# DanielPS555/Radix-sort-Merge-Sort-CUDA---Lab-y-practicos-GPGPU-2023

Hardware: AMD Instinct MI355X
Metric: Mkeys/s sorting uint32, n=2^28, 1 GPU (+ merge-sort at 2/4/8) (higher is better)
Workload: dtype u32; 1 GPU; LSD radix sort (8-bit digits, onesweep), n=2^28 uint32 u32, device-resident (BASELINE config 3); n_per_gpu=268435456, algo=radix, key=u32, dist=u32, parallelism=single GPU

## Files before the change

### radix-sort-merge-sort-cuda---lab-y-practicos-gpgpu-2023_amd/csrc/api.hip

```cpp
#include <hip/hip_runtime.h>

#include <algorithm>
#include <cstdio>
#include <cstdlib>
#include <cstring>
#include <mutex>
#include <vector>

#include "host.h"
#include "segsort.h"

using namespace labsort;

namespace {

thread_local int g_last_hip = 0;

struct TimedLaunch {
    int cls;
    hipEvent_t a, b;
};
std::mutex g_timing_mu;
bool g_timing_on = false;
std::vector<TimedLaunch> g_pending;
// ... 100 lines not shown

bool use_gather(size_t n) {
    const char *e = std::getenv("LABSORT_RADIX_IMPL");
    if (e && !std::strcmp(e, "gather")) return true;
    if (n < GS_MIN_N || n >= GS_MAX_N) return false;
    return !(e && !std::strcmp(e, "onesweep"));
}

uint32_t hybrid_gate(size_t n) {
    const char *e = std::getenv("LABSORT_RADIX_HYBRID");
    if (e && !std::strcmp(e, "0")) return 0u;
    if (e && !std::strcmp(e, "2")) return HY_MAX_BUCKET;
    return n >= HY_MIN_N && n <= HY_MAX_N ? HY_FAST_GROUP : 0u;
}

uint32_t hy_count_mode() {
    const char *e = std::getenv("LABSORT_HY_COUNT");
    if (e && !std::strcmp(e, "lean")) return HY_COUNT_LEAN;
    if (e && !std::strcmp(e, "full")) return HY_COUNT_FULL;
    return HY_COUNT_AUTO;
}

bool small_path(size_t n, int algo) { return algo != LABSORT_ALGO_RADIX1 && n <= (size_t)TS_TILE; }

int sort_radix8(const uint32_t *ki, const uint32_t *vi, uint32_t *ko, uint32_t *vo, size_t n, uint32_t flip, char *ws,
                hipStream_t s) {
    const RadixLayout L = radix_layout(n, 8, OSP_TILE);
    Bufs b, vb;
    b.p[SEL_IN] = const_cast<uint32_t *>(ki);
    b.p[SEL_OUT] = ko;
    b.p[SEL_TMP] = reinterpret_cast<uint32_t *>(ws + L.off_tmp);
    vb.p[SEL_IN] = const_cast<uint32_t *>(vi);
    vb.p[SEL_OUT] = vo;
    vb.p[SEL_TMP] = vi ? reinterpret_cast<uint32_t *>(ws + align_up(L.total, 256)) : nullptr;
    uint32_t *hist = reinterpret_cast<uint32_t *>(ws + L.off_hist);
    uint32_t *counters = reinterpret_cast<uint32_t *>(ws + L.off_counter);
    uint32_t *err = reinterpret_cast<uint32_t *>(ws + L.off_err);
    uint32_t *lookback = reinterpret_cast<uint32_t *>(ws + L.off_lookback);
    Plan *plan = reinterpret_cast<Plan *>(ws + L.off_plan);
    HIP_TRY(launch_zero(ws, L.off_lookback, s));
    uint32_t *hps = reinterpret_cast<uint32_t *>(ws + L.off_hps);
    uint32_t *joint = reinterpret_cast<uint32_t *>(ws + L.off_joint);
    SegPlan *sps = reinterpret_cast<SegPlan *>(ws + L.off_segplan);
    const uint32_t hy_limit = vi ? 0u : hybrid_gate(n);
    const bool hyb = hy_limit != 0u;
    const HyCounts hc{reinterpret_cast<uint32_t *>(ws + L.off_hps2), reinterpret_cast<uint32_t *>(ws + L.off_top14), hy_limit,
                      err, hy_count_mode()};
    {
        TimingScope ts(LABSORT_K_HISTOGRAM, s);
        if (hyb) HIP_TRY(launch_hist_lean(ki, n, flip, joint, s, hc));
        HIP_TRY(launch_hist_seg(ki, n, flip, hps, joint, s, hyb ? &hc : nullptr));
    }
    HIP_TRY(launch_plan8(hps, joint, n, ki == ko ? 1 : 0, plan, sps, hist, ws + L.off_lookback,
                         L.zero_bytes - L.off_lookback, s, hyb ? &hc : nullptr));
    for (int p = 0; p < L.P; ++p) {
        TimingScope ts(hyb && p < 2 ? LABSORT_K_UNTIMED : LABSORT_K_ONESWEEP, s);
        HIP_TRY(launch_onesweep_p(b, plan, p, n, flip, sps + p, lookback + (size_t)p * L.ntiles * L.R,
                                  counters + (size_t)p * OSP_NCTR, err, s, vi ? &vb : nullptr));
    }
    if (hyb) {
        TimingScope ts(LABSORT_K_SEGSORT, s);
        HIP_TRY(launch_hybrid_finish(plan, b, n, flip, hist, sps + 3, lookback + (size_t)3 * L.ntiles * L.R, L.ntiles, err,
                                     reinterpret_cast<uint32_t *>(ws + L.off_fin_hdr),
                                     reinterpret_cast<uint32_t *>(ws + L.off_fin_off),
                                     reinterpret_cast<uint32_t *>(ws + L.off_fin_lists), s));
    }
    if (ki == ko) {
        HIP_TRY(launch_final_copy(b, plan, n, s));
        if (vi) HIP_TRY(launch_final_copy(vb, plan, n, s));
    }
    return LABSORT_OK;
}

int sort_radix1(const uint32_t *in, uint32_t *out, size_t n, uint32_t flip, char *ws, hipStream_t s) {
    const RadixLayout L = radix_layout(n, 1, OS_TILE);
    Bufs b;
    b.p[SEL_IN] = const_cast<uint32_t *>(in);
    b.p[SEL_OUT] = out;
    b.p[SEL_TMP] = reinterpret_cast<uint32_t *>(ws + L.off_tmp);
    uint32_t *hist = reinterpret_cast<uint32_t *>(ws + L.off_hist);
    uint32_t *counters = reinterpret_cast<uint32_t *>(ws + L.off_counter);
    uint32_t *err = reinterpret_cast<uint32_t *>(ws + L.off_err);
    uint32_t *lookback = reinterpret_cast<uint32_t *>(ws + L.off_lookback);
    Plan *plan = reinterpret_cast<Plan *>(ws + L.off_plan);
    HIP_TRY(launch_zero(ws, L.zero_bytes, s));
    {
        TimingScope ts(LABSORT_K_HISTOGRAM, s);
        HIP_TRY(launch_histogram(in, n, flip, 1, hist, s));
    }
    HIP_TRY(launch_plan(hist, n, 1, in == out ? 1 : 0, plan, s));
    for (int p = 0; p < L.P; ++p) {
        TimingScope ts(LABSORT_K_ONESWEEP, s);
        HIP_TRY(launch_onesweep(b, plan, p, 1, n, flip, hist, lookback + (size_t)p * L.ntiles * L.R,
                                counters + (size_t)p * OSP_NCTR, err, s));
    }
    HIP_TRY(launch_final_copy(b, plan, n, s));
    return LABSORT_OK;
}

int sort_merge(const uint32_t *ki, const uint32_t *vi, uint32_t *ko, uint32_t *vo, size_t n, uint32_t flip, char *ws,
               hipStream_t s) {
    const bool pairs = vi != nullptr;
    const MergeLayout L = merge_layout(n, pairs);
    uint32_t *err = reinterpret_cast<uint32_t *>(ws + L.off_err);
    HIP_TRY(launch_zero(err, 16, s));
    uint32_t *tk = reinterpret_cast<uint32_t *>(ws + L.off_tk);
    uint32_t *tv = pairs ? reinterpret_cast<uint32_t *>(ws + L.off_tv) : nullptr;
// ... 595 lines not shown
```

### radix-sort-merge-sort-cuda---lab-y-practicos-gpgpu-2023_amd/csrc/common.h

```cpp
#pragma once
#include <hip/hip_runtime.h>
#include <stddef.h>
#include <stdint.h>

namespace labsort {

constexpr int WAVE = 64;

__host__ __device__ inline uint32_t f32_ord(uint32_t x) {
    if ((x & 0x7FFFFFFFu) > 0x7F800000u) return 0xFFFFFFFFu;
    return (x & 0x80000000u) ? ~x : x | 0x80000000u;
}
__host__ __device__ inline uint32_t f32_unord(uint32_t o) { return (o & 0x80000000u) ? o & 0x7FFFFFFFu : ~o; }

constexpr uint32_t BF16_NAN_T = 0x7F80u, F16_NAN_T = 0x7C00u;
__host__ __device__ inline uint32_t ord16(uint32_t x, uint32_t nan_t) {
    x &= 0xFFFFu;
    if ((x & 0x7FFFu) > nan_t) return 0xFFFFu;
    return (x & 0x8000u) ? ~x & 0xFFFFu : x | 0x8000u;
}
__host__ __device__ inline uint32_t unord16(uint32_t o) { return (o & 0x8000u) ? o & 0x7FFFu : ~o & 0xFFFFu; }

constexpr int RADIX_BITS = 8;
constexpr int OS_BLOCK = 512;
// ... 81 lines not shown

constexpr int HY_TOP_BITS = 14, HY_TOP = 1 << HY_TOP_BITS;
constexpr uint32_t HY_BUCKETS = 1u << 16;
constexpr uint32_t HY_MAX_BUCKET = 32768;
constexpr size_t HY_MIN_N = ((size_t)1 << 28) - ((size_t)1 << 24);
constexpr size_t HY_MAX_N = ((size_t)1 << 28) + 3 * ((size_t)1 << 24);
constexpr uint32_t HY_FAST_GROUP = 4u * 5120u;
struct HyCounts {
    uint32_t *hps2;
    uint32_t *top14;
    uint32_t limit;
    uint32_t *ctl;
    uint32_t mode;
};
constexpr uint32_t HY_CTL_TICKET = 1;
constexpr uint32_t HY_CTL_NAND = 2;
constexpr uint32_t HY_CTL_OR = 3;
constexpr uint32_t HY_CTL_VERDICT = 4;
constexpr uint32_t HY_CTL_LEAN = 5;
constexpr uint32_t HY_CTL_FULL = 6;
constexpr uint32_t HY_VERDICT_CLASSIC = 1, HY_VERDICT_HYBRID = 2;
constexpr uint32_t HY_COUNT_AUTO = 0, HY_COUNT_LEAN = 1, HY_COUNT_FULL = 2;
#ifndef LABSORT_HY_LEAN_SL
#define LABSORT_HY_LEAN_SL 32
#endif
constexpr int HY_LEAN_SL = LABSORT_HY_LEAN_SL;
inline uint32_t hist_seg_bps(size_t n) {
    const size_t bps = n / ((size_t)NSEG * HS_MIN_KEYS);
    return (uint32_t)(bps < 1 ? 1 : bps > (size_t)HS_BPS ? (size_t)HS_BPS : bps);
}

struct Bufs {
    uint32_t *p[3];
};

constexpr uint32_t LB_AGG = 1u << 30;
constexpr uint32_t LB_INC = 2u << 30;
constexpr uint32_t LB_VAL = (1u << 30) - 1u;
constexpr size_t RADIX_MAX_N = (size_t)LB_VAL;

hipError_t launch_fill(uint32_t *out, size_t n, uint64_t seed, int dist, uint64_t param, uint64_t first,
                       hipStream_t s);
hipError_t launch_histogram(const uint32_t *keys, size_t n, uint32_t flip, int bits, uint32_t *hist,
                            hipStream_t s);
hipError_t launch_plan(const uint32_t *hist, size_t n, int bits, int in_is_out, Plan *plan, hipStream_t s);
hipError_t launch_onesweep(Bufs b, const Plan *plan, int pass, int bits, size_t n, uint32_t flip,
                           const uint32_t *hist, uint32_t *lookback, uint32_t *counter, uint32_t *err,
                           hipStream_t s);
hipError_t launch_hist_seg(const uint32_t *keys, size_t n, uint32_t flip, uint32_t *hps, uint32_t *joint,
                           hipStream_t s, const HyCounts *hy = nullptr);
hipError_t launch_hist_lean(const uint32_t *keys, size_t n, uint32_t flip, uint32_t *joint, hipStream_t s,
                            const HyCounts &hy);
hipError_t launch_plan8(const uint32_t *hps, const uint32_t *joint, size_t n, int in_is_out, Plan *plan,
                        SegPlan *segplans, uint32_t *hist, void *zero_p, size_t zero_bytes, hipStream_t s,
                        const HyCounts *hy = nullptr);
hipError_t launch_onesweep_p(Bufs b, const Plan *plan, int pass, size_t n, uint32_t flip, const SegPlan *sp,
                             uint32_t *lookback, uint32_t *counter, uint32_t *err, hipStream_t s,
                             const Bufs *vb = nullptr);
hipError_t launch_final_copy(Bufs b, const Plan *plan, size_t n, hipStream_t s);
hipError_t launch_tile_sort(const uint32_t *in, uint32_t *out, size_t n, uint32_t flip, hipStream_t s,
                            uint32_t *samp_out = nullptr);
hipError_t launch_wave_tile_sort(uint32_t *keys, size_t n, uint32_t flip, hipStream_t s);
hipError_t launch_merge_pass(const uint32_t *in, uint32_t *out, size_t n, size_t run, uint32_t flip,
                             hipStream_t s, const uint32_t *vin = nullptr, uint32_t *vout = nullptr,
                             const MgPairs *pairs = nullptr, uint32_t *samp_out = nullptr);
hipError_t launch_tile_sort_kv(const uint32_t *in, uint32_t *out, const uint32_t *vin, uint32_t *vout, size_t n,
                               uint32_t flip, hipStream_t s, uint32_t *samp_out = nullptr);
#ifndef LABSORT_M4_S
#define LABSORT_M4_S 128
#endif
constexpr uint32_t M4_S = LABSORT_M4_S;
inline size_t merge4_samp_words(size_t n) { return (n + M4_S - 1) / M4_S + 4; }
size_t merge4_bnd_words(size_t n, size_t r);
hipError_t launch_merge4_pass(const uint32_t *in, uint32_t *out, size_t n, size_t r, uint32_t flip, uint32_t *bnd,
                              const uint32_t *samp_in, uint32_t *samp_out, hipStream_t s, const uint32_t *vin = nullptr,
                              uint32_t *vout = nullptr, uint32_t *err = nullptr);
hipError_t launch_merge_ab(const uint32_t *a, size_t la, const uint32_t *b, size_t lb, uint32_t *out, size_t d0,
                           size_t d1, uint32_t flip, uint32_t *part, hipStream_t s);
hipError_t launch_upper_bound(const uint32_t *keys, size_t n, uint32_t flip, const uint32_t *values, size_t nv,
                              uint32_t *out, hipStream_t s);
struct KeyPrint {
    uint64_t s1, s2, x;
};
bool verify_enabled();
KeyPrint key_print(const int *a, size_t n);
void verify_or_exit(const char *who, const int *a, size_t n, const KeyPrint &before);

hipError_t launch_zero(void *p, size_t bytes, hipStream_t s);
hipError_t launch_stream_copy(const uint32_t *in, uint32_t *out, size_t n, hipStream_t s);
hipError_t launch_f32_map(const uint32_t *in, uint32_t *out, size_t n, bool inverse, hipStream_t s);
hipError_t launch_count_descents(const uint32_t *keys, size_t n, uint32_t flip, uint32_t *count, hipStream_t s);

}
```

### radix-sort-merge-sort-cuda---lab-y-practicos-gpgpu-2023_amd/csrc/fin_block.h

```cpp
#pragma once
#include "segsort.h"

#include "devutil.h"

namespace labsort {

namespace {

#ifndef LABSORT_FIN_PREFETCH
#define LABSORT_FIN_PREFETCH 1
#endif

__device__ __forceinline__ uint32_t wave_incl_scan_dpp(uint32_t x) {
    x += (uint32_t)__builtin_amdgcn_update_dpp(0, (int)x, 0x111, 0xf, 0xf, false);
    x += (uint32_t)__builtin_amdgcn_update_dpp(0, (int)x, 0x112, 0xf, 0xf, false);
    x += (uint32_t)__builtin_amdgcn_update_dpp(0, (int)x, 0x114, 0xf, 0xf, false);
    x += (uint32_t)__builtin_amdgcn_update_dpp(0, (int)x, 0x118, 0xf, 0xf, false);
    x += (uint32_t)__builtin_amdgcn_update_dpp(0, (int)x, 0x142, 0xa, 0xf, false);
    x += (uint32_t)__builtin_amdgcn_update_dpp(0, (int)x, 0x143, 0xc, 0xf, false);
    return x;
}

template <int BLOCK, int KPT>
struct FinSmem {
    static constexpr int R = 256, W = BLOCK / WAVE, TILE = BLOCK * KPT;
    static_assert(TILE <= 65536, "16-bit LDS slots");
    static_assert(W == 4, "the fold holds one counter row per wave in registers");
    uint32_t keys[TILE];
    alignas(16) uint32_t cnt[W * R];
    alignas(16) uint32_t offs[W * R];
    uint32_t probe[WAVE];
    uint32_t ordered;
};

struct FinStripe {
    size_t sb;
    uint32_t ws0;
    uint32_t nf;
    uint32_t ng;
    bool tail_ok;
};
template <int W, int KPT>
__device__ __forceinline__ FinStripe fin_stripe(uint32_t b, uint32_t len, uint32_t lane, uint32_t wid) {
    if (len > (uint32_t)(W * WAVE * KPT)) len = 0u;
    const uint32_t jn = (len + (uint32_t)(W * WAVE) - 1u) / (uint32_t)(W * WAVE);
    const uint32_t ws0 = wid * jn * WAVE;
    const uint32_t rem = ws0 < len ? len - ws0 : 0u;
    const uint32_t nf = min(jn, rem / WAVE);
    const uint32_t tail = nf < jn ? rem - nf * WAVE : 0u;
    return {(size_t)b + ws0, ws0, nf, nf + (tail ? 1u : 0u), lane < tail};
}

template <int KPT>
__device__ __forceinline__ void fin_load(const uint32_t *in, const FinStripe &g, uint32_t lane, uint32_t (&k)[KPT]) {
    const char *pb = reinterpret_cast<const char *>(in + g.sb);
    const uint32_t lb = lane * 4u;
    if (g.nf == (uint32_t)KPT) {
#pragma unroll
        for (int j = 0; j < KPT; ++j) k[j] = ld_stream<NT_TILE>(reinterpret_cast<const uint32_t *>(pb + (lb + (uint32_t)(j * WAVE * 4))));
    } else {
#pragma unroll
        for (int j = 0; j < KPT; ++j) {
            k[j] = 0xFFFFFFFFu;
            if ((uint32_t)j < g.nf || ((uint32_t)j == g.nf && g.tail_ok))
                k[j] = ld_stream<NT_TILE>(reinterpret_cast<const uint32_t *>(pb + (lb + (uint32_t)(j * WAVE * 4))));
        }
    }
}

template <int BLOCK, int KPT>
__device__ __forceinline__ void fin_pass(FinSmem<BLOCK, KPT> &sm, const uint32_t (&k)[KPT], uint32_t shift, uint32_t ng,
                                         bool atomic_rank, uint32_t lane, uint32_t wid) {
    constexpr int W = FinSmem<BLOCK, KPT>::W, R = FinSmem<BLOCK, KPT>::R;
    uint32_t *wh = sm.cnt + wid * R;
    uint32_t *wo = sm.offs + wid * R;
    uint32_t n0 = ng, n1 = ng;
    asm volatile("" : "+s"(n0), "+s"(n1));
    uint32_t z = 0u;
    asm volatile("" : "+v"(z));
    *reinterpret_cast<uint4 *>(wh + 4u * lane) = make_uint4(z, z, z, z);
    uint32_t rank[KPT / 2] = {};
#pragma unroll
    for (int j = 0; j < KPT; ++j) {
        uint32_t r = 0u;
        if ((uint32_t)j < n0) r = rank8(wh, (k[j] >> shift) & 0xFFu, lane, atomic_rank);
        set16(rank, j, r);
    }
    __syncthreads();
    {
        uint4 c[W];
#pragma unroll
        for (int w = 0; w < W; ++w) c[w] = *reinterpret_cast<const uint4 *>(sm.cnt + w * R + 4u * lane);
        uint32_t tot[4] = {0u, 0u, 0u, 0u}, bef[4] = {0u, 0u, 0u, 0u};
#pragma unroll
        for (int w = 0; w < W; ++w) {
            const uint32_t cw[4] = {c[w].x, c[w].y, c[w].z, c[w].w};
            const bool before = (uint32_t)w < wid;
#pragma unroll
            for (int q = 0; q < 4; ++q) {
                tot[q] += cw[q];
                bef[q] += before ? cw[q] : 0u;
            }
        }
        const uint32_t s = tot[0] + tot[1] + tot[2] + tot[3];
        uint32_t run = wave_incl_scan_dpp(s) - s;
        uint4 o4;
        o4.x = run + bef[0];
        run += tot[0];
        o4.y = run + bef[1];
        run += tot[1];
        o4.z = run + bef[2];
        run += tot[2];
        o4.w = run + bef[3];
        *reinterpret_cast<uint4 *>(wo + 4u * lane) = o4;
    }
    __builtin_amdgcn_wave_barrier();
#pragma unroll
    for (int j = 0; j < KPT; ++j)
        if ((uint32_t)j < n1) set16(rank, j, wo[(k[j] >> shift) & 0xFFu] + get16(rank, j));
#pragma unroll
    for (int j = 0; j < KPT; ++j)
        if ((uint32_t)j < n1) sm.keys[get16(rank, j)] = k[j];
    __syncthreads();
}

template <int BLOCK, int KPT, int WPE>
__global__ __launch_bounds__(BLOCK, WPE) void k_fin_block(uint32_t *out, const uint32_t *__restrict__ off,
                                                           const uint32_t *__restrict__ hdr,
                                                           const uint32_t *__restrict__ list, HySel hy) {
    using S = FinSmem<BLOCK, KPT>;
    constexpr int W = S::W;
    constexpr int CLS = 3;
    constexpr bool PREFETCH = LABSORT_FIN_PREFETCH != 0;
    __shared__ S sm;
    if (hy.plan->hybrid == 0u) return;
    const uint32_t *in = hy.buf[hy.plan->fin_src];
    if (ld_agent(hdr) != 0u) return;
    const uint32_t cnt = hdr[SEG_HDR_CNT + CLS];
    const uint32_t tid = threadIdx.x, lane = tid & 63u, wid = __builtin_amdgcn_readfirstlane(tid >> 6);
    if (blockIdx.x >= cnt) return;
    probe_lane_order(sm.probe, &sm.ordered, lane, wid);
    __syncthreads();
    const bool atomic_rank = lane_order_probed(&sm.ordered);
    uint32_t nb, ne;
    {
        const uint32_t seg = __builtin_amdgcn_readfirstlane(list[blockIdx.x]);
        nb = __builtin_amdgcn_readfirstlane(off[seg]);
        ne = __builtin_amdgcn_readfirstlane(off[seg + 1]);
    }
    uint32_t k[KPT];
    FinStripe g = fin_stripe<W, KPT>(nb, ne - nb, lane, wid);
    if constexpr (PREFETCH) fin_load(in, g, lane, k);
    for (uint32_t it = blockIdx.x; it < cnt; it += gridDim.x) {
        if constexpr (!PREFETCH) {
            g = fin_stripe<W, KPT>(nb, ne - nb, lane, wid);
            fin_load(in, g, lane, k);
        }
        const bool more = it + gridDim.x < cnt;
        if (more) {
            const uint32_t seg = __builtin_amdgcn_readfirstlane(list[it + gridDim.x]);
            nb = __builtin_amdgcn_readfirstlane(off[seg]);
            ne = __builtin_amdgcn_readfirstlane(off[seg + 1]);
        }
        fin_pass(sm, k, 0u, g.ng, atomic_rank, lane, wid);
        {
            uint32_t n2 = g.ng;
            asm volatile("" : "+s"(n2));
#pragma unroll
            for (int j = 0; j < KPT; ++j)
                if ((uint32_t)j < n2) k[j] = sm.keys[g.ws0 + (uint32_t)j * WAVE + lane];
        }
        fin_pass(sm, k, 8u, g.ng, atomic_rank, lane, wid);
        FinStripe gn = g;
        uint32_t kn[PREFETCH ? KPT : 1];
        if constexpr (PREFETCH) {
            gn = fin_stripe<W, KPT>(nb, more ? ne - nb : 0u, lane, wid);
            fin_load(in, gn, lane, kn);
        }
        uint32_t nfs = g.nf;
        asm volatile("" : "+s"(nfs));
        const uint32_t *sk = sm.keys + g.ws0 + lane;
        char *ob = reinterpret_cast<char *>(out + g.sb);
        const uint32_t lb = lane * 4u;
        if (nfs == (uint32_t)KPT) {
#pragma unroll
            for (int j = 0; j < KPT; ++j) *reinterpret_cast<uint32_t *>(ob + (lb + (uint32_t)(j * WAVE * 4))) = sk[j * WAVE];
        } else {
#pragma unroll
            for (int j = 0; j < KPT; ++j)
                if ((uint32_t)j < nfs || ((uint32_t)j == nfs && g.tail_ok))
                    *reinterpret_cast<uint32_t *>(ob + (lb + (uint32_t)(j * WAVE * 4))) = sk[j * WAVE];
        }
        if constexpr (PREFETCH) {
            g = gn;
#pragma unroll
            for (int j = 0; j < KPT; ++j) k[j] = kn[j];
        }
    }
}

}

}
```

### radix-sort-merge-sort-cuda---lab-y-practicos-gpgpu-2023_amd/csrc/kernels.hip

```cpp
#include "common.h"
#include "devutil.h"
#include "host.h"
#include "lds_pass.h"

#include <cstdlib>
#include <cstring>
#include <type_traits>

namespace labsort {

__device__ __forceinline__ uint64_t mix64(uint64_t z) {
    z += 0x9E3779B97F4A7C15ull;
    z = (z ^ (z >> 30)) * 0xBF58476D1CE4E5B9ull;
    z = (z ^ (z >> 27)) * 0x94D049BB133111EBull;
    return z ^ (z >> 31);
}

__global__ __launch_bounds__(256) void k_fill(uint32_t *__restrict__ out, size_t n, uint64_t seed, int dist,
                                              uint64_t param, uint64_t first) {
    const size_t stride = (size_t)gridDim.x * blockDim.x;
    for (size_t i = (size_t)blockIdx.x * blockDim.x + threadIdx.x; i < n; i += stride) {
        const uint64_t gi = first + i;
        const uint64_t z = mix64(seed ^ (gi * 0x9E3779B97F4A7C15ull));
        const uint32_t hi = (uint32_t)(z >> 32);
// ... 259 lines not shown
__device__ void build_segplan(SegPlan *__restrict__ sp, const uint32_t *__restrict__ hs, const uint32_t *start,
                              uint32_t mode, uint32_t *sh ) {
    const uint32_t t = threadIdx.x;
    uint32_t tot = 0;
    for (int s = 0; s < NSEG; ++s) {
        const uint32_t v = hs[s * 256 + t];
        sh[s * 256 + t] = v;
        tot += v;
    }
    uint32_t run = block_excl_scan<256, 256>(tot, sh + NSEG * 256);
    for (int s = 0; s < NSEG; ++s) {
        sp->base[s * 256 + t] = run;
        run += sh[s * 256 + t];
    }
    if (t <= (uint32_t)NSEG) sp->start[t] = start[t];
    if (t == 0) {
        uint32_t tp = 0, mx = 0;
        for (int s = 0; s <= NSEG; ++s) {
            sp->tpre[s] = tp;
            if (s < NSEG) {
                const uint32_t a0 = start[s] - start[s] % (uint32_t)OSP_TILE;
                const uint32_t ts = start[s + 1] > start[s] ? (start[s + 1] - a0 + OSP_TILE - 1) / OSP_TILE : 0u;
                tp += ts;
                mx = ts > mx ? ts : mx;
            }
        }
        sp->maxt = mx;
        sp->mode = mode;
        sp->segbits = mode == 2u ? 0u : 4u;
    }
}

__device__ void build_segplan_later(SegPlan *__restrict__ out, int q, uint32_t prev, uint32_t n, int seg_later,
                                    const uint32_t *hist, const uint32_t *__restrict__ joint, uint32_t *sh,
                                    uint32_t *start) {
    const uint32_t t = threadIdx.x;
    if (seg_later <= 0 || prev + 1u != (uint32_t)q) {
        for (int s = 0; s < NSEG; ++s) sh[s * 256 + t] = s ? 0u : hist[q * 256 + t];
        if (t <= (uint32_t)NSEG) start[t] = t ? n : 0u;
        __syncthreads();
        build_segplan(out, sh, start, 2u, sh);
        return;
    }
    const uint32_t ex = block_excl_scan<256, 256>(hist[prev * 256 + t], sh + NSEG * 256);
    if ((t & 15u) == 0) start[t >> 4] = ex;
    if (t == 0) start[NSEG] = n;
    __syncthreads();
    build_segplan(out, joint + (size_t)q * NSEG * 256, start, 1u, sh);
}

__global__ __launch_bounds__(256) void k_plan8(const uint32_t *__restrict__ hps, const uint32_t *__restrict__ joint,
                                               uint32_t n, int in_is_out, int seg_later, Plan *__restrict__ plan,
                                               SegPlan *__restrict__ sps, uint32_t *__restrict__ hist_out,
                                               uint4 *__restrict__ zp, size_t zn4, HyCounts hy) {
    constexpr uint32_t PW = 4;
    if (blockIdx.x >= PW) {
        const size_t stride = (size_t)(gridDim.x - PW) * blockDim.x;
        for (size_t i = (size_t)(blockIdx.x - PW) * blockDim.x + threadIdx.x; i < zn4; i += stride)
            zp[i] = make_uint4(0u, 0u, 0u, 0u);
        return;
    }
    const int me = (int)blockIdx.x;
    __shared__ uint32_t hist[4 * 256];
    __shared__ uint32_t sh[NSEG * 256 + 8];
    __shared__ uint32_t triv[4];
    __shared__ uint32_t start[NSEG + 1];
    __shared__ uint32_t prevs[4];
    __shared__ int first;
    __shared__ uint32_t max14;
    const uint32_t t = threadIdx.x;
    if (t < 4) triv[t] = 0;
    if (t == 0) max14 = 0u;
    __syncthreads();
    const uint32_t verdict = hy.ctl ? hy.ctl[HY_CTL_VERDICT] : 0u;
    if (hy.top14 && verdict == 0u) {
        uint32_t m = 0;
        for (uint32_t i = t; i < (uint32_t)HY_TOP; i += 256u) m = max(m, hy.top14[i]);
        atomicMax(&max14, m);
    }
    uint32_t v[4] = {0, 0, 0, 0};
    for (int s = 0; s < NSEG; ++s) {
        v[0] += hps[s * 256 + t];
#pragma unroll
        for (int p = 1; p < 4; ++p) v[p] += joint[(p * NSEG + s) * 256 + t];
    }
#pragma unroll
    for (int p = 0; p < 4; ++p) {
        hist[p * 256 + t] = v[p];
        if (me == 0) hist_out[p * 256 + t] = v[p];
        if (v[p] == n) triv[p] = 1;
    }
    if (t <= (uint32_t)NSEG) start[t] = seg_later < 0 ? (t ? n : 0u) : seg_start(t, n);
    __syncthreads();
    const bool hybrid = verdict ? verdict == HY_VERDICT_HYBRID
                                : hy.top14 && !triv[0] && !triv[1] && max14 <= min(hy.limit, HY_MAX_BUCKET);
    __syncthreads();
    if (hybrid && t < 2) triv[t] = 1;
    __syncthreads();
    if (t == 0 && me != 0) {
        int k = 0, last = -1;
        for (int p = 0; p < 4; ++p) {
            prevs[p] = NEXT_NONE;
            if (!triv[p]) {
                if (last >= 0) prevs[p] = (uint32_t)last;
                last = p;
                if (!k++) first = p;
            }
        }
        if (!k) first = -1;
    }
    if (t == 0 && me == 0) {
// ... 1059 lines not shown
    k_fill<<<blocks_for(n, 256 * 8, 8192), 256, 0, s>>>(out, n, seed, dist, param, first);
    return hipGetLastError();
}

hipError_t launch_histogram(const uint32_t *keys, size_t n, uint32_t flip, int bits, uint32_t *hist,
                            hipStream_t s) {
    if (n == 0) return hipSuccess;
    const unsigned g = blocks_for(n, 16384, 256);
    if (bits == 8) k_histogram<8><<<g, HIST_BLOCK, 0, s>>>(keys, n, flip, hist);
    else if (bits == 1) k_histogram<1><<<g, HIST_BLOCK, 0, s>>>(keys, n, flip, hist);
    else return hipErrorInvalidValue;
    return hipGetLastError();
}

hipError_t launch_plan(const uint32_t *hist, size_t n, int bits, int in_is_out, Plan *plan, hipStream_t s) {
    k_plan<<<1, 256, 0, s>>>(hist, (uint32_t)n, bits, in_is_out, plan);
    return hipGetLastError();
}

hipError_t launch_onesweep(Bufs b, const Plan *plan, int pass, int bits, size_t n, uint32_t flip,
                           const uint32_t *hist, uint32_t *lookback, uint32_t *counter, uint32_t *err,
                           hipStream_t s) {
    if (bits != 1) return hipErrorInvalidValue;
    const unsigned g = (unsigned)((n + OS_TILE - 1) / OS_TILE);
    k_onesweep<1, OS_BLOCK, OS_KPT><<<g, OS_BLOCK, 0, s>>>(b, plan, pass, (uint32_t)n, flip, hist, lookback, counter,
                                                           err);
    return hipGetLastError();
}

hipError_t launch_onesweep_p(Bufs b, const Plan *plan, int pass, size_t n, uint32_t flip, const SegPlan *sp,
                             uint32_t *lookback, uint32_t *counter, uint32_t *err, hipStream_t s, const Bufs *vb) {
    if (n > RADIX_MAX_N) return hipErrorInvalidValue;
    const size_t ntiles = (n + OSP_TILE - 1) / OSP_TILE + NSEG;
    const size_t want = (size_t)cu_count();
    const unsigned g = (unsigned)(ntiles < want ? ntiles : want);
    if (vb)
        k_onesweep_p<true><<<g, OSP_KV_BLOCK, 0, s>>>(b, plan, pass, (uint32_t)n, flip, sp, lookback, counter, err, *vb);
    else
        k_onesweep_p<false><<<g, OSP_BLOCK, 0, s>>>(b, plan, pass, (uint32_t)n, flip, sp, lookback, counter, err, b);
    return hipGetLastError();
}


hipError_t launch_hist_seg(const uint32_t *keys, size_t n, uint32_t flip, uint32_t *hps, uint32_t *joint,
                           hipStream_t s, const HyCounts *hy) {
    if (n == 0) return hipSuccess;
    const uint32_t bps = hist_seg_bps(n);
    if (hy) k_hist_seg<true><<<NSEG * (unsigned)bps, HIST_BLOCK, 0, s>>>(keys, n, flip, hps, joint, (uint32_t)bps, *hy);
    else k_hist_seg<false><<<NSEG * (unsigned)bps, HIST_BLOCK, 0, s>>>(keys, n, flip, hps, joint, (uint32_t)bps, HyCounts{});
    return hipGetLastError();
}

hipError_t launch_plan8(const uint32_t *hps, const uint32_t *joint, size_t n, int in_is_out, Plan *plan,
                        SegPlan *segplans, uint32_t *hist, void *zero_p, size_t zero_bytes, hipStream_t s,
                        const HyCounts *hy) {
    const bool fold = zero_bytes % 16 == 0;
    if (!fold && zero_bytes) {
        const hipError_t z = launch_zero(zero_p, zero_bytes, s);
        if (z != hipSuccess) return z;
    }
    const size_t zn4 = fold ? zero_bytes / 16 : 0;
    const unsigned g = 4u + (zn4 ? blocks_for(zn4, 256 * 4, 2048) : 0u);
    k_plan8<<<g, 256, 0, s>>>(hps, joint, (uint32_t)n, in_is_out, 1, plan, segplans, hist,
                              static_cast<uint4 *>(zero_p), zn4, hy ? *hy : HyCounts{});
    return hipGetLastError();
}


__global__ __launch_bounds__(256) void k_zero(uint4 *__restrict__ p4, size_t n4, uint32_t *__restrict__ tail,
                                             uint32_t ntail) {
    const size_t stride = (size_t)gridDim.x * blockDim.x;
    for (size_t i = (size_t)blockIdx.x * blockDim.x + threadIdx.x; i < n4; i += stride) p4[i] = make_uint4(0, 0, 0, 0);
    if (blockIdx.x == 0 && threadIdx.x < ntail) tail[threadIdx.x] = 0u;
}

hipError_t launch_zero(void *p, size_t bytes, hipStream_t s) {
    if (bytes == 0) return hipSuccess;
    const size_t n4 = bytes / 16;
    uint32_t *tail = reinterpret_cast<uint32_t *>(static_cast<char *>(p) + n4 * 16);
    const uint32_t ntail = (uint32_t)((bytes - n4 * 16) / 4);
    k_zero<<<blocks_for(n4 ? n4 : 1, 256 * 4, 2048), 256, 0, s>>>(static_cast<uint4 *>(p), n4, tail, ntail);
    return hipGetLastError();
}

hipError_t launch_final_copy(Bufs b, const Plan *plan, size_t n, hipStream_t s) {
    k_final_copy<<<blocks_for(n, 256 * 16, 4096), 256, 0, s>>>(b, plan, n);
    return hipGetLastError();
}

hipError_t launch_tile_sort(const uint32_t *in, uint32_t *out, size_t n, uint32_t flip, hipStream_t s,
                            uint32_t *samp_out) {
    if (n == 0) return hipSuccess;
    const size_t nt = (n + TS_TILE - 1) / TS_TILE;
    k_tile_sort<TS_KBLOCK, TS_KPT><<<(unsigned)nt, TS_KBLOCK, 0, s>>>(in, out, nullptr, nullptr, (uint32_t)n, flip,
                                                                     samp_out);
    return hipGetLastError();
}

hipError_t launch_wave_tile_sort(uint32_t *keys, size_t n, uint32_t flip, hipStream_t s) {
    if (n == 0) return hipSuccess;
    const unsigned g = (unsigned)((n + 255) / 256);
    k_wave_split<<<g, 256, 0, s>>>(keys, (uint32_t)n, flip);
    return hipGetLastError();
}

hipError_t launch_merge_pass(const uint32_t *in, uint32_t *out, size_t n, size_t run, uint32_t flip,
                             hipStream_t s, const uint32_t *vin, uint32_t *vout, const MgPairs *pairs,
                             uint32_t *samp_out) {
    MgPairs pr{};
    if (pairs) pr = *pairs;
    if (n == 0) return hipSuccess;
    const uint32_t ntiles = (uint32_t)((n + MG_TILE - 1) / MG_TILE);
    const uint32_t want = (uint32_t)(MG_BLOCKS_PER_CU * cu_count());
    uint32_t m = (ntiles + want - 1) / want;
    if (m > (uint32_t)MG_MAX_TPB) m = MG_MAX_TPB;
    const uint32_t g = (ntiles + m - 1) / m;
    if (vin)
// ... 73 lines not shown
```

### radix-sort-merge-sort-cuda---lab-y-practicos-gpgpu-2023_amd/csrc/segsort.h

```cpp
#pragma once
#include <type_traits>

#include "common.h"

namespace labsort {

#ifndef LABSORT_SEG_WAVE_KPT
#define LABSORT_SEG_WAVE_KPT 4
#endif
#ifndef LABSORT_SEG_WAVE2_KPT
#define LABSORT_SEG_WAVE2_KPT 8
#endif
#ifndef LABSORT_SEG_WAVE3_KPT
#define LABSORT_SEG_WAVE3_KPT 16
#endif
constexpr int SEG_WAVE_KPT = LABSORT_SEG_WAVE_KPT, SEG_WAVE2_KPT = LABSORT_SEG_WAVE2_KPT,
              SEG_WAVE3_KPT = LABSORT_SEG_WAVE3_KPT;
constexpr int SEG_WAVE_KEYS = WAVE * SEG_WAVE_KPT, SEG_WAVE2_KEYS = WAVE * SEG_WAVE2_KPT,
              SEG_WAVE3_KEYS = WAVE * SEG_WAVE3_KPT;
static_assert(SEG_WAVE_KEYS < SEG_WAVE2_KEYS && SEG_WAVE2_KEYS < SEG_WAVE3_KEYS, "class edges ascend");
constexpr int SEG_WAVE_WPB = 4;
#ifndef LABSORT_SEG_BLOCK
#define LABSORT_SEG_BLOCK 256
#endif
#ifndef LABSORT_SEG_BLOCK_KPT
#define LABSORT_SEG_BLOCK_KPT 16
#endif
#ifndef LABSORT_SEG_BLOCK_WGS
#define LABSORT_SEG_BLOCK_WGS 6
#endif
#ifndef LABSORT_SEG_BLOCK_WPE
#define LABSORT_SEG_BLOCK_WPE 4
#endif
constexpr int SEG_BLOCK_WPE = LABSORT_SEG_BLOCK_WPE;
constexpr int SEG_BLOCK = LABSORT_SEG_BLOCK;
constexpr int SEG_BLOCK_KPT = LABSORT_SEG_BLOCK_KPT;
constexpr int SEG_BLOCK_WGS = LABSORT_SEG_BLOCK_WGS;
constexpr int SEG_BLOCK_KEYS = SEG_BLOCK * SEG_BLOCK_KPT;
constexpr int SEG_TILE_KEYS = TS_BLOCK * TS_KPT;
constexpr int SEG_TILE_PAIRS = TS_BLOCK * TS_KPT_KV;
constexpr int SEG_CLASSES = 5;
struct SegEdges {
    uint32_t e[SEG_CLASSES - 1];
};
static_assert(SEG_WAVE3_KEYS < SEG_BLOCK_KEYS, "class edges ascend");
struct SegClass {
    int keys;
    int block;
    int kpt, kpt_kv;
    int wpe;
    int wgs, wgs_kv;
};
constexpr SegClass SEG_CLASS[SEG_CLASSES] = {
    {SEG_WAVE_KEYS, SEG_WAVE_WPB * WAVE, SEG_WAVE_KPT, SEG_WAVE_KPT, 0, 8, 8},
    {SEG_WAVE2_KEYS, SEG_WAVE_WPB * WAVE, SEG_WAVE2_KPT, SEG_WAVE2_KPT, 0, 8, 6},
    {SEG_WAVE3_KEYS, SEG_WAVE_WPB * WAVE, SEG_WAVE3_KPT, SEG_WAVE3_KPT, 0, 4, 4},
    {SEG_BLOCK_KEYS, SEG_BLOCK, SEG_BLOCK_KPT, SEG_BLOCK_KPT, SEG_BLOCK_WPE, SEG_BLOCK_WGS, 4},
    {SEG_TILE_KEYS, TS_BLOCK, TS_KPT, TS_KPT_KV, 4, 1, 1},
};
inline int seg_class_of(size_t len) {
    int c = 0;
    while (c < SEG_CLASSES - 1 && len > (size_t)SEG_CLASS[c].keys) ++c;
    return c;
}
template <int C = 0, class Fn>
hipError_t seg_class_dispatch(int c, Fn &&fn) {
    if constexpr (C < SEG_CLASSES) return c == C ? fn(std::integral_constant<int, C>{}) : seg_class_dispatch<C + 1>(c, fn);
    else return hipErrorInvalidValue;
}

constexpr int SEG_HDR_BYTES = 256;
constexpr int SEG_HDR_DEVERR = 1, SEG_HDR_CNT = 4;

hipError_t launch_seg_bin(const uint32_t *off, size_t nseg, size_t n, size_t max_len, bool pairs, bool copy1,
                          uint32_t *hdr, uint32_t *lists, size_t stride, hipStream_t s);
hipError_t launch_seg_lds_classes(size_t max_len, bool pairs, const uint32_t *in, uint32_t *out, const uint32_t *vin,
                                  uint32_t *vout, const uint32_t *off, const uint32_t *hdr, const uint32_t *lists,
                                  size_t stride, uint32_t flip, bool f32, hipStream_t s);
struct HySel {
    const Plan *plan;
    const uint32_t *buf[3];
};
constexpr int HY_BLOCK = 256, HY_BLOCK_KPT = 20, HY_BLOCK_WPE = 5, HY_BLOCK_KEYS = HY_BLOCK * HY_BLOCK_KPT;
static_assert((uint32_t)SEG_TILE_KEYS == HY_MAX_BUCKET, "the plan's bound is the tile class's capacity");
static_assert(SEG_WAVE3_KEYS < HY_BLOCK_KEYS && HY_BLOCK_KEYS < SEG_TILE_KEYS, "class edges ascend");
static_assert(HY_FAST_GROUP == 4u * HY_BLOCK_KEYS, "the default gate's group bound: four block-class buckets");
hipError_t launch_hybrid_finish(const Plan *plan, Bufs b, size_t n, uint32_t flip, const uint32_t *hist, const SegPlan *sp3,
                                const uint32_t *lookback3, size_t nslots, uint32_t *err, uint32_t *hdr, uint32_t *off,
                                uint32_t *lists, hipStream_t s);

size_t seg_inner_bytes(size_t n);

}
```

### radix-sort-merge-sort-cuda---lab-y-practicos-gpgpu-2023_amd/csrc/segsort.hip

```cpp
#include "segsort.h"

#include <algorithm>

#include "devutil.h"
#include "fin_block.h"
#include "host.h"
#include "seg_kernels.h"

namespace labsort {

namespace {

constexpr int BIN_BLOCK = 1024, BIN_SPT = 4;

__global__ __launch_bounds__(BIN_BLOCK) void k_seg_bin(const uint32_t *__restrict__ off, uint32_t nseg, uint32_t n,
                                                        uint32_t max_len, SegEdges e, uint32_t copy1,
                                                        uint32_t *__restrict__ hdr, uint32_t *__restrict__ lists,
                                                        size_t stride, const Plan *__restrict__ hyplan) {
    __shared__ uint32_t cnt[SEG_CLASSES], base[SEG_CLASSES];
    if (hyplan && hyplan->hybrid == 0u) return;
    const uint32_t tid = threadIdx.x, lane = tid & 63u;
    if (tid < (uint32_t)SEG_CLASSES) cnt[tid] = 0u;
    __syncthreads();
    uint32_t cls[BIN_SPT], pos[BIN_SPT];
// ... 175 lines not shown
}

__global__ __launch_bounds__(FE_BLOCK) void k_fin_edges(const Plan *__restrict__ plan, Bufs bufs, uint32_t n, uint32_t flip,
                                                        const uint32_t *__restrict__ hist, const SegPlan *__restrict__ sp,
                                                        const uint32_t *__restrict__ lb, uint32_t nslots, uint32_t *err,
                                                        uint32_t *hdr, uint32_t *__restrict__ off) {
    __shared__ uint32_t wh[FE_W * 256];
    __shared__ uint32_t wsum[4];
    __shared__ uint32_t s2;
    if (plan->hybrid == 0u) return;
    const uint32_t tid = threadIdx.x, d2 = blockIdx.x;
    const uint32_t h2 = tid < 256u ? hist[2 * 256 + tid] : 0u;
    const uint32_t x2 = block_excl_scan<FE_BLOCK, 256>(h2, wsum);
    if (tid == d2) s2 = min(x2, n);
    __syncthreads();
    const uint32_t P = s2;
    uint32_t o;
    bool bad = false;
    if (plan->src[3] == SEL_SKIP) {
        const uint32_t h3 = tid < 256u ? hist[3 * 256 + tid] : 0u;
        o = block_excl_scan<FE_BLOCK, 256>(h3, wsum) + (h3 == n ? P : 0u);
    } else {
        o = fin_edge_at(P, bufs.p[plan->src[3]], flip, sp, lb, nslots, wh, bad);
    }
    if (tid >= 256u) return;
    if (bad) {
        atomicOr(err, 1u);
        atomicOr(hdr, 1u);
        return;
    }
    const uint32_t q = (tid << 8) | d2;
    off[q] = o;
    if (q == HY_BUCKETS - 1u) off[HY_BUCKETS] = n;
}
}

hipError_t launch_hybrid_finish(const Plan *plan, Bufs b, size_t n, uint32_t flip, const uint32_t *hist, const SegPlan *sp3,
                                const uint32_t *lookback3, size_t nslots, uint32_t *err, uint32_t *hdr, uint32_t *off,
                                uint32_t *lists, hipStream_t s) {
    const size_t stride = HY_BUCKETS;
    k_fin_edges<<<256, FE_BLOCK, 0, s>>>(plan, b, (uint32_t)n, flip, hist, sp3, lookback3, (uint32_t)nslots, err, hdr, off);
    hipError_t e = hipGetLastError();
    if (e != hipSuccess) return e;
    const SegEdges ed{{(uint32_t)SEG_WAVE_KEYS, (uint32_t)SEG_WAVE2_KEYS, (uint32_t)SEG_WAVE3_KEYS, (uint32_t)HY_BLOCK_KEYS}};
    k_seg_bin<<<HY_BUCKETS / (BIN_BLOCK * BIN_SPT), BIN_BLOCK, 0, s>>>(off, HY_BUCKETS, (uint32_t)n, HY_MAX_BUCKET, ed, 1u, hdr,
                                                                      lists, stride, plan);
    if ((e = hipGetLastError()) != hipSuccess) return e;
    const HySel hy{plan, {b.p[0], b.p[1], b.p[2]}};
    uint32_t *out = b.p[SEL_OUT];
    const unsigned cus = (unsigned)cu_count();
    for (int c = 0; c < SEG_CLASSES; ++c) {
        const uint32_t *list = lists + (size_t)c * stride;
        if (c == 3) {
            k_fin_block<HY_BLOCK, HY_BLOCK_KPT, HY_BLOCK_WPE><<<cus * (unsigned)HY_BLOCK_WPE, HY_BLOCK, 0, s>>>(out, off, hdr, list, hy);
            e = hipGetLastError();
        } else {
            e = launch_seg_sort(c, out, out, nullptr, nullptr, off, hdr, list, flip, s, hy);
        }
        if (e != hipSuccess) return e;
    }
    return hipSuccess;
}

size_t seg_inner_bytes(size_t n) {
    const size_t m = n < (size_t)LABSORT_AUTO_PAIRS_MERGE_MAX_KEYS ? n : (size_t)LABSORT_AUTO_PAIRS_MERGE_MAX_KEYS;
    return std::max(labsort_pairs_workspace_bytes(n, LABSORT_ALGO_AUTO), labsort_pairs_workspace_bytes(m, LABSORT_ALGO_MERGE));
}

}

using namespace labsort;

extern "C" {

size_t labsort_segment_tile_keys(void) { return (size_t)SEG_TILE_KEYS; }
size_t labsort_segment_pair_tile_keys(void) { return (size_t)SEG_TILE_PAIRS; }

int labsort_segment_class_edges(int pairs, size_t *edges, int cap) {
    const size_t e[SEG_CLASSES] = {(size_t)SEG_WAVE_KEYS, (size_t)SEG_WAVE2_KEYS, (size_t)SEG_WAVE3_KEYS, (size_t)SEG_BLOCK_KEYS,
                                   pairs ? (size_t)SEG_TILE_PAIRS : (size_t)SEG_TILE_KEYS};
    for (int i = 0; i < SEG_CLASSES && i < cap && edges; ++i) edges[i] = e[i];
    return SEG_CLASSES;
}

namespace {
bool seg_lds_path(size_t max_len, int pairs) {
    return max_len > 0 && max_len <= (pairs ? (size_t)SEG_TILE_PAIRS : (size_t)SEG_TILE_KEYS);
}
struct SegLayout {
    size_t off_lists, list_stride;
    size_t off_a, off_b, off_c, off_inner, inner_bytes;
    size_t total;
};
SegLayout seg_layout(size_t n, size_t nseg, bool lds) {
    SegLayout L{};
    Carver c{SEG_HDR_BYTES};
    if (lds) {
        L.list_stride = align_up(nseg * 4, 256) / 4;
        L.off_lists = c.take((size_t)SEG_CLASSES * L.list_stride * 4);
        L.total = c.o;
    } else {
        L.off_a = c.take(n * 4);
        L.off_b = c.take(n * 4);
        L.off_c = c.take(n * 4);
        L.off_inner = c.o;
        L.inner_bytes = seg_inner_bytes(n);
        L.total = c.o + L.inner_bytes;
// ... 99 lines not shown
```

Measured before the change: 154,500 Mkeys/s.

## Use atomic ticket work-stealing in block-class finish and skip redundant lookback zeroing

The block-class segment-sort kernel drops its static grid-stride bucket assignment and pulls work dynamically from a global atomic ticket held in the cleared segment header, granting several buckets per draw. The draw is overlapped with the current bucket's sort, with double-buffered shared slots. The aim is to balance uneven bucket sizes across blocks and cut tail imbalance, at the cost of extra atomics. Separately, the plan kernel skips zeroing the first two passes' look-back regions when the hybrid verdict holds, since those passes are not used in that path, which cuts memset traffic.

```diff
diff --git a/radix-sort-merge-sort-cuda---lab-y-practicos-gpgpu-2023_amd/csrc/api.hip b/radix-sort-merge-sort-cuda---lab-y-practicos-gpgpu-2023_amd/csrc/api.hip
--- a/radix-sort-merge-sort-cuda---lab-y-practicos-gpgpu-2023_amd/csrc/api.hip
+++ b/radix-sort-merge-sort-cuda---lab-y-practicos-gpgpu-2023_amd/csrc/api.hip
@@ -176,7 +176,7 @@
         HIP_TRY(launch_hist_seg(ki, n, flip, hps, joint, s, hyb ? &hc : nullptr));
     }
     HIP_TRY(launch_plan8(hps, joint, n, ki == ko ? 1 : 0, plan, sps, hist, ws + L.off_lookback,
-                         L.zero_bytes - L.off_lookback, s, hyb ? &hc : nullptr));
+                         L.zero_bytes - L.off_lookback, L.ntiles * L.R * 4, s, hyb ? &hc : nullptr));
     for (int p = 0; p < L.P; ++p) {
         TimingScope ts(hyb && p < 2 ? LABSORT_K_UNTIMED : LABSORT_K_ONESWEEP, s);
         HIP_TRY(launch_onesweep_p(b, plan, p, n, flip, sps + p, lookback + (size_t)p * L.ntiles * L.R,
diff --git a/radix-sort-merge-sort-cuda---lab-y-practicos-gpgpu-2023_amd/csrc/common.h b/radix-sort-merge-sort-cuda---lab-y-practicos-gpgpu-2023_amd/csrc/common.h
--- a/radix-sort-merge-sort-cuda---lab-y-practicos-gpgpu-2023_amd/csrc/common.h
+++ b/radix-sort-merge-sort-cuda---lab-y-practicos-gpgpu-2023_amd/csrc/common.h
@@ -157,8 +157,8 @@
 hipError_t launch_hist_lean(const uint32_t *keys, size_t n, uint32_t flip, uint32_t *joint, hipStream_t s,
                             const HyCounts &hy);
 hipError_t launch_plan8(const uint32_t *hps, const uint32_t *joint, size_t n, int in_is_out, Plan *plan,
-                        SegPlan *segplans, uint32_t *hist, void *zero_p, size_t zero_bytes, hipStream_t s,
-                        const HyCounts *hy = nullptr);
+                        SegPlan *segplans, uint32_t *hist, void *zero_p, size_t zero_bytes, size_t pass_bytes,
+                        hipStream_t s, const HyCounts *hy = nullptr);
 hipError_t launch_onesweep_p(Bufs b, const Plan *plan, int pass, size_t n, uint32_t flip, const SegPlan *sp,
                              uint32_t *lookback, uint32_t *counter, uint32_t *err, hipStream_t s,
                              const Bufs *vb = nullptr);
diff --git a/radix-sort-merge-sort-cuda---lab-y-practicos-gpgpu-2023_amd/csrc/fin_block.h b/radix-sort-merge-sort-cuda---lab-y-practicos-gpgpu-2023_amd/csrc/fin_block.h
--- a/radix-sort-merge-sort-cuda---lab-y-practicos-gpgpu-2023_amd/csrc/fin_block.h
+++ b/radix-sort-merge-sort-cuda---lab-y-practicos-gpgpu-2023_amd/csrc/fin_block.h
@@ -10,6 +10,11 @@
 #ifndef LABSORT_FIN_PREFETCH
 #define LABSORT_FIN_PREFETCH 1
 #endif
+#ifndef LABSORT_FIN_GRANT
+#define LABSORT_FIN_GRANT 4
+#endif
+constexpr int FIN_GRANT = LABSORT_FIN_GRANT;
+static_assert(FIN_GRANT >= 1, "a ticket grants at least one entry");
 
 __device__ __forceinline__ uint32_t wave_incl_scan_dpp(uint32_t x) {
     x += (uint32_t)__builtin_amdgcn_update_dpp(0, (int)x, 0x111, 0xf, 0xf, false);
@@ -31,6 +36,7 @@
     alignas(16) uint32_t offs[W * R];
     uint32_t probe[WAVE];
     uint32_t ordered;
+    uint32_t tick[2];
 };
 
 struct FinStripe {
@@ -127,7 +133,7 @@
 template <int BLOCK, int KPT, int WPE>
 __global__ __launch_bounds__(BLOCK, WPE) void k_fin_block(uint32_t *out, const uint32_t *__restrict__ off,
                                                            const uint32_t *__restrict__ hdr,
-                                                           const uint32_t *__restrict__ list, HySel hy) {
+                                                           const uint32_t *__restrict__ list, uint32_t *ticket, HySel hy) {
     using S = FinSmem<BLOCK, KPT>;
     constexpr int W = S::W;
     constexpr int CLS = 3;
@@ -139,9 +145,13 @@
     const uint32_t cnt = hdr[SEG_HDR_CNT + CLS];
     const uint32_t tid = threadIdx.x, lane = tid & 63u, wid = __builtin_amdgcn_readfirstlane(tid >> 6);
     if (blockIdx.x >= cnt) return;
+    const bool any_more = cnt > gridDim.x;
+    if (any_more && tid == 0u) sm.tick[1] = __hip_atomic_fetch_add(ticket, 1u, __ATOMIC_RELAXED, __HIP_MEMORY_SCOPE_AGENT);
     probe_lane_order(sm.probe, &sm.ordered, lane, wid);
     __syncthreads();
     const bool atomic_rank = lane_order_probed(&sm.ordered);
+    uint32_t nxt = any_more ? gridDim.x + (uint32_t)FIN_GRANT * __builtin_amdgcn_readfirstlane(sm.tick[1]) : cnt;
+    uint32_t left = (uint32_t)FIN_GRANT - 1u;
     uint32_t nb, ne;
     {
         const uint32_t seg = __builtin_amdgcn_readfirstlane(list[blockIdx.x]);
@@ -151,14 +161,17 @@
     uint32_t k[KPT];
     FinStripe g = fin_stripe<W, KPT>(nb, ne - nb, lane, wid);
     if constexpr (PREFETCH) fin_load(in, g, lane, k);
-    for (uint32_t it = blockIdx.x; it < cnt; it += gridDim.x) {
+    for (uint32_t it = blockIdx.x, par = 0u; it < cnt; par ^= 1u) {
         if constexpr (!PREFETCH) {
             g = fin_stripe<W, KPT>(nb, ne - nb, lane, wid);
             fin_load(in, g, lane, k);
         }
-        const bool more = it + gridDim.x < cnt;
+        const bool more = nxt < cnt;
+        const bool draw = more && (FIN_GRANT == 1 || left == 0u);
+        uint32_t drawn = 0u;
+        if (draw && tid == 0u) drawn = __hip_atomic_fetch_add(ticket, 1u, __ATOMIC_RELAXED, __HIP_MEMORY_SCOPE_AGENT);
         if (more) {
-            const uint32_t seg = __builtin_amdgcn_readfirstlane(list[it + gridDim.x]);
+            const uint32_t seg = __builtin_amdgcn_readfirstlane(list[nxt]);
             nb = __builtin_amdgcn_readfirstlane(off[seg]);
             ne = __builtin_amdgcn_readfirstlane(off[seg + 1]);
         }
@@ -170,7 +183,16 @@
             for (int j = 0; j < KPT; ++j)
                 if ((uint32_t)j < n2) k[j] = sm.keys[g.ws0 + (uint32_t)j * WAVE + lane];
         }
+        if (draw && tid == 0u) sm.tick[par] = drawn;
         fin_pass(sm, k, 8u, g.ng, atomic_rank, lane, wid);
+        it = nxt;
+        if (draw) {
+            nxt = gridDim.x + (uint32_t)FIN_GRANT * __builtin_amdgcn_readfirstlane(sm.tick[par]);
+            left = (uint32_t)FIN_GRANT - 1u;
+        } else {
+            nxt += 1u;
+            left -= 1u;
+        }
         FinStripe gn = g;
         uint32_t kn[PREFETCH ? KPT : 1];
         if constexpr (PREFETCH) {
diff --git a/radix-sort-merge-sort-cuda---lab-y-practicos-gpgpu-2023_amd/csrc/kernels.hip b/radix-sort-merge-sort-cuda---lab-y-practicos-gpgpu-2023_amd/csrc/kernels.hip
--- a/radix-sort-merge-sort-cuda---lab-y-practicos-gpgpu-2023_amd/csrc/kernels.hip
+++ b/radix-sort-merge-sort-cuda---lab-y-practicos-gpgpu-2023_amd/csrc/kernels.hip
@@ -335,11 +335,13 @@
 __global__ __launch_bounds__(256) void k_plan8(const uint32_t *__restrict__ hps, const uint32_t *__restrict__ joint,
                                                uint32_t n, int in_is_out, int seg_later, Plan *__restrict__ plan,
                                                SegPlan *__restrict__ sps, uint32_t *__restrict__ hist_out,
-                                               uint4 *__restrict__ zp, size_t zn4, HyCounts hy) {
+                                               uint4 *__restrict__ zp, size_t zn4, size_t zr4, HyCounts hy) {
     constexpr uint32_t PW = 4;
     if (blockIdx.x >= PW) {
         const size_t stride = (size_t)(gridDim.x - PW) * blockDim.x;
-        for (size_t i = (size_t)(blockIdx.x - PW) * blockDim.x + threadIdx.x; i < zn4; i += stride)
+        const bool lean_hybrid = hy.ctl && hy.ctl[HY_CTL_VERDICT] == HY_VERDICT_HYBRID;
+        const size_t first = lean_hybrid ? min(2 * zr4, zn4) : (size_t)0;
+        for (size_t i = first + (size_t)(blockIdx.x - PW) * blockDim.x + threadIdx.x; i < zn4; i += stride)
             zp[i] = make_uint4(0u, 0u, 0u, 0u);
         return;
     }
@@ -1505,9 +1507,9 @@
 }
 
 hipError_t launch_plan8(const uint32_t *hps, const uint32_t *joint, size_t n, int in_is_out, Plan *plan,
-                        SegPlan *segplans, uint32_t *hist, void *zero_p, size_t zero_bytes, hipStream_t s,
-                        const HyCounts *hy) {
-    const bool fold = zero_bytes % 16 == 0;
+                        SegPlan *segplans, uint32_t *hist, void *zero_p, size_t zero_bytes, size_t pass_bytes,
+                        hipStream_t s, const HyCounts *hy) {
+    const bool fold = zero_bytes % 16 == 0 && pass_bytes % 16 == 0 && zero_bytes == 4 * pass_bytes;
     if (!fold && zero_bytes) {
         const hipError_t z = launch_zero(zero_p, zero_bytes, s);
         if (z != hipSuccess) return z;
@@ -1515,7 +1517,7 @@
     const size_t zn4 = fold ? zero_bytes / 16 : 0;
     const unsigned g = 4u + (zn4 ? blocks_for(zn4, 256 * 4, 2048) : 0u);
     k_plan8<<<g, 256, 0, s>>>(hps, joint, (uint32_t)n, in_is_out, 1, plan, segplans, hist,
-                              static_cast<uint4 *>(zero_p), zn4, hy ? *hy : HyCounts{});
+                              static_cast<uint4 *>(zero_p), zn4, pass_bytes / 16, hy ? *hy : HyCounts{});
     return hipGetLastError();
 }
 
diff --git a/radix-sort-merge-sort-cuda---lab-y-practicos-gpgpu-2023_amd/csrc/segsort.h b/radix-sort-merge-sort-cuda---lab-y-practicos-gpgpu-2023_amd/csrc/segsort.h
--- a/radix-sort-merge-sort-cuda---lab-y-practicos-gpgpu-2023_amd/csrc/segsort.h
+++ b/radix-sort-merge-sort-cuda---lab-y-practicos-gpgpu-2023_amd/csrc/segsort.h
@@ -70,7 +70,8 @@
 }
 
 constexpr int SEG_HDR_BYTES = 256;
-constexpr int SEG_HDR_DEVERR = 1, SEG_HDR_CNT = 4;
+constexpr int SEG_HDR_DEVERR = 1, SEG_HDR_CNT = 4, SEG_HDR_TICKET = SEG_HDR_CNT + SEG_CLASSES;
+static_assert((SEG_HDR_TICKET + 1) * 4 <= SEG_HDR_BYTES, "the ticket lies inside the cleared header");
 
 hipError_t launch_seg_bin(const uint32_t *off, size_t nseg, size_t n, size_t max_len, bool pairs, bool copy1,
                           uint32_t *hdr, uint32_t *lists, size_t stride, hipStream_t s);
diff --git a/radix-sort-merge-sort-cuda---lab-y-practicos-gpgpu-2023_amd/csrc/segsort.hip b/radix-sort-merge-sort-cuda---lab-y-practicos-gpgpu-2023_amd/csrc/segsort.hip
--- a/radix-sort-merge-sort-cuda---lab-y-practicos-gpgpu-2023_amd/csrc/segsort.hip
+++ b/radix-sort-merge-sort-cuda---lab-y-practicos-gpgpu-2023_amd/csrc/segsort.hip
@@ -251,7 +251,8 @@
     for (int c = 0; c < SEG_CLASSES; ++c) {
         const uint32_t *list = lists + (size_t)c * stride;
         if (c == 3) {
-            k_fin_block<HY_BLOCK, HY_BLOCK_KPT, HY_BLOCK_WPE><<<cus * (unsigned)HY_BLOCK_WPE, HY_BLOCK, 0, s>>>(out, off, hdr, list, hy);
+            k_fin_block<HY_BLOCK, HY_BLOCK_KPT, HY_BLOCK_WPE><<<cus * (unsigned)HY_BLOCK_WPE, HY_BLOCK, 0, s>>>(
+                out, off, hdr, list, hdr + SEG_HDR_TICKET, hy);
             e = hipGetLastError();
         } else {
             e = launch_seg_sort(c, out, out, nullptr, nullptr, off, hdr, list, flip, s, hy);
```

Measured after the change: 157,600 Mkeys/s, median of 6. +2.1%, better.
